# Coda-Research-Group/LearnedMetricIndex

Hardware: AMD Instinct MI355X
Metric: queries/sec @ recall@10, 768-d 10M index, 10k query batch (higher is better)
Workload: dtype f16 prefilter (f32 accumulate) + f32 exact re-rank; outputs identical to the all-f32 path

## Files before the change

learnedmetricindex_amd/csrc/lmi_handle.h:

```cpp
#pragma once
#include <hip/hip_runtime_api.h>

#include <cstdarg>
#include <cstdint>
#include <cstdio>
#include <string>
#include <utility>
#include <vector>

namespace {

thread_local std::string g_err;

int fail(const char* fmt, ...) {
    char buf[1024];
    va_list ap;
    va_start(ap, fmt);
    vsnprintf(buf, sizeof(buf), fmt, ap);
    va_end(ap);
    g_err = buf;
    return -1;
}

#define HIPCHK(expr)                                                                                \
// ... 152 lines not shown
    DevBuf aug_rows, q_aug, qn2;
    DevBuf stage;
    DevBuf wide;
    DevBuf q16_nav, q16_srch;
    bool q_srch_async = false;
    DevBuf rd_flag;
    DevBuf qdelta, qnorm, qscale, qfrag16, eps2, cand_cnt, cand_row, cand_s, fallback, pf_bound, nkeep, surv_row, rs_flag, rs_active;
    DevBuf grp_scratch;
    DevBuf x_log, x_ext, x_off, fb_list;
    unsigned x_cap = 0;
    DevBuf redo;
    size_t stamps_off = 0;
    int last_nslots = 0, last_nb = 0;
    long long last_ncols = 0;
    bool last_fast = false;
    static constexpr int PLAN_WORDS = 32;
    int32_t last_plan[PLAN_WORDS] = {};
    int32_t last_mlp_plan[PLAN_WORDS] = {};
    DevBuf act[2], xfrag, logits, order, q_nav, q_srch;
    DevBuf m, cb_start, item_base, part_base, stats, head, slot_local, slot_col, colmap, qfrag, grp, col_thr;
    DevBuf part_score, part_row, rank_d, rank_id, out_d, out_id, out_key;
    static constexpr int EV_RING = 128;
    hipEvent_t ev_ring[EV_RING][10] = {};
    bool valid_ring[EV_RING][10] = {};
    int ev_cur = 0;
    long long ev_calls = 0;
    hipEvent_t* ev = ev_ring[0];
    bool* ev_valid = valid_ring[0];
    long long h_stats[4] = {0, 0, 0, 0};
    bool stats_pending = false;
    DevBuf ts_ring;
    unsigned ts_mask[EV_RING] = {};
    unsigned long long* ts_set = nullptr;
    DevBuf fr_dbg;
    DevBuf cb_alloc, cb_bucket;
    unsigned* h_oflag = nullptr;
    int overflow_armed = 0;
    bool fr_bump_pending = false;
    DevBuf mut_pos, mut_ids, mut_list, mut_keep, mut_src, mut_stage, mut_word;
    lmi_index* parent = nullptr;
    int live_clones = 0;
};

struct lmi_index : DeviceFacts, Settings, Switches, Models, Buckets, CallState {};

static lmi_index* clone_handle(lmi_index* h) {
    lmi_index* c = new lmi_index();
    static_cast<DeviceFacts&>(*c) = *h;
    static_cast<Settings&>(*c) = *h;
    static_cast<Switches&>(*c) = *h;
    static_cast<Models&>(*c) = *h;
    static_cast<Buckets&>(*c) = *h;
    c->parent = h;
    h->live_clones++;
    return c;
}
```

learnedmetricindex_amd/csrc/lmi_host_debug.h:

```cpp
#pragma once
#include "lmi_host_mutate.h"
#include "lmi_host_search.h"

static int read_event_set(const hipEvent_t* ev, const bool* ev_valid, float* ms) {
    for (int i = 0; i < LMI_T_COUNT; ++i) ms[i] = 0.0f;
    auto span = [&](int a, int b, float* out) -> int {
        if (ev_valid[a] && ev_valid[b]) HIPCHK(hipEventElapsedTime(out, ev[a], ev[b]));
        return 0;
    };
    CHK(span(0, 1, &ms[LMI_T_INFERENCE]));
    CHK(span(1, 2, &ms[LMI_T_ROUTE]));
    CHK(span(2, 3, &ms[LMI_T_SCAN]));
    CHK(span(3, 4, &ms[LMI_T_MERGE]));
    CHK(span(2, 5, &ms[LMI_T_PF_SAMPLE]));
    CHK(span(5, 6, &ms[LMI_T_PF_EMIT]));
    CHK(span(6, 7, &ms[LMI_T_RESCORE]));
    CHK(span(7, 3, &ms[LMI_T_FALLBACK]));
    int first = ev_valid[0] ? 0 : 1;
    int last = ev_valid[4] ? 4 : 1;
    CHK(span(first, last, &ms[LMI_T_TOTAL]));
    return 0;
}

static void read_stamp_set(const lmi_index* h, const unsigned long long* v, unsigned mask, float* ms) {
// ... 154 lines not shown
    if (!h) return fail("lmi_debug_read_candidates: NULL handle");
    if (!h->last_fast) return fail("lmi_debug_read_candidates: the last scan did not use the prefilter");
    if (slot < 0 || slot >= h->last_nslots) return fail("lmi_debug_read_candidates: slot outside the last scan's %d", h->last_nslots);
    CHK(set_dev(h));
    HIPCHK(hipStreamSynchronize(h->stream));
    int col = -1;
    HIPCHK(hipMemcpy(&col, h->slot_col.as<int>() + slot, 4, hipMemcpyDeviceToHost));
    unsigned cnt = 0;
    float e2 = 0.0f, qs = 1.0f, xs[2] = {1.0f, 1.0f};
    if (col >= 0) {
        HIPCHK(hipMemcpy(&cnt, h->cand_cnt.as<unsigned>() + col, 4, hipMemcpyDeviceToHost));
        HIPCHK(hipMemcpy(&e2, h->eps2.as<float>() + col, 4, hipMemcpyDeviceToHost));
        HIPCHK(hipMemcpy(&qs, h->qscale.as<float>() + slot / h->last_nb, 4, hipMemcpyDeviceToHost));
        HIPCHK(hipMemcpy(xs, h->xscale.p, 8, hipMemcpyDeviceToHost));
        const unsigned n = std::min<unsigned>(std::min<unsigned>(cnt, (unsigned)PF_CAP), (unsigned)std::max(cap, 0));
        if (n && rows) HIPCHK(hipMemcpy(rows, h->cand_row.as<unsigned>() + (size_t)col * PF_CAP, (size_t)n * 4, hipMemcpyDeviceToHost));
        if (n && shat) HIPCHK(hipMemcpy(shat, h->cand_s.as<float>() + (size_t)col * PF_CAP, (size_t)n * 4, hipMemcpyDeviceToHost));
    }
    if (count) *count = col >= 0 ? (int)cnt : -1;
    if (eps2) *eps2 = e2;
    if (qscale) *qscale = qs;
    if (xscale) *xscale = xs[0];
    return 0;
}

extern "C" LMI_API int lmi_debug_peek(lmi_index* h, const char* name, void* dst, int64_t bytes) {
    if (!h || !name || !dst) return fail("lmi_debug_peek: NULL argument");
    CHK(set_dev(h));
    HIPCHK(hipStreamSynchronize(h->stream));
    DevBuf* b = nullptr;
    size_t off = 0;
    if (!strcmp(name, "pf_bound")) b = &h->pf_bound;
    if (!strcmp(name, "fr_dbg")) b = &h->fr_dbg;
    if (!strcmp(name, "pf_stamps")) { b = &h->pf_bound; off = h->stamps_off; }
    if (!strcmp(name, "cand_total")) {
        if (bytes != 8 || !h->last_fast) return fail("lmi_debug_peek: cand_total is 8 bytes after a prefilter scan");
        unsigned long long* d_acc = reinterpret_cast<unsigned long long*>(h->stats.as<long long>() + 2);
        HIPCHK(hipMemsetAsync(d_acc, 0, 8, h->stream));
        sum_u32_kernel<<<64, 256, 0, h->stream>>>(h->cand_cnt.as<unsigned>(), h->last_ncols, d_acc);
        HIPCHK(hipGetLastError());
        HIPCHK(hipStreamSynchronize(h->stream));
        HIPCHK(hipMemcpy(dst, d_acc, 8, hipMemcpyDeviceToHost));
        return 0;
    }
    if (!strcmp(name, "pf_redo")) b = &h->redo;
    if (!strcmp(name, "pf_fallback")) b = &h->fb_list;
    if (!b) return fail("lmi_debug_peek: unknown buffer '%s'", name);
    if (bytes < 0 || off + (size_t)bytes > b->cap) return fail("lmi_debug_peek: %lld bytes asked of a %zu-byte buffer", (long long)bytes, b->cap);
    if (bytes) HIPCHK(hipMemcpy(dst, static_cast<char*>(b->p) + off, (size_t)bytes, hipMemcpyDeviceToHost));
    return 0;
}

extern "C" LMI_API int lmi_scan_stats(lmi_index* h, double* flops, int64_t* pairs, int64_t* items) {
    if (!h) return fail("lmi_scan_stats: NULL handle");
    CHK(set_dev(h));
    if (h->stats_pending) {
        HIPCHK(hipStreamSynchronize(h->stream));
        HIPCHK(hipMemcpy(h->h_stats, h->stats.p, 32, hipMemcpyDeviceToHost));
        h->stats_pending = false;
    }
    if (pairs) *pairs = h->h_stats[0];
    if (items) *items = h->h_stats[1];
    if (flops) *flops = 2.0 * h->d * (double)h->h_stats[0];
    return 0;
}
```

learnedmetricindex_amd/csrc/lmi_host_model.h:

```cpp
#pragma once
#include "lmi_host.h"

static int pack_from_host(lmi_index* h, const float* src, int rows, int cols, int n_rb, int KG, DevBuf& dst) {
    CHK(h->stage.reserve((size_t)rows * cols * sizeof(float)));
    HIPCHK(hipMemcpyAsync(h->stage.p, src, (size_t)rows * cols * sizeof(float), hipMemcpyHostToDevice, h->stream));
    CHK(dst.reserve((size_t)n_rb * KG * 1024));
    long long total = (long long)n_rb * 32 * KG;
    pack_gather_kernel<<<cdiv(total, 256), 256, 0, h->stream>>>(h->stage.as<float>(), cols, nullptr, rows,
                                                               (long long)n_rb * 32, KG, dst.as<float4>());
    HIPCHK(hipGetLastError());
    HIPCHK(hipStreamSynchronize(h->stream));
    return 0;
}

static int pack_model(lmi_index* h, const char* who, int n_layers, const int* dims, const float* const* W, const float* const* b, Model& m) {
    h->desc_dirty = true;
    m.n_layers = 0;
    if (n_layers < 1 || n_layers > LMI_MAX_LAYERS) return fail("%s: n_layers %d out of range", who, n_layers);
    for (int i = 0; i <= n_layers; ++i)
        if (dims[i] < 1) return fail("%s: dims[%d] = %d", who, i, dims[i]);
    m.dims.assign(dims, dims + n_layers + 1);
    m.n_rb.assign(n_layers, 0);
    m.KG.assign(n_layers, 0);
    m.Wf.assign(n_layers, DevBuf());
// ... 134 lines not shown
        HIPCHK(hipMemcpy(h->d_child_model.p, child_model, (size_t)total * 4, hipMemcpyHostToDevice));
        HIPCHK(hipMemcpy(h->d_child_bucket.p, child_bucket, (size_t)total * 4, hipMemcpyHostToDevice));
    }
    h->tree_set = true;
    return 0;
}

struct FusedLds {
    bool ok = true;
    bool logits_lds = true;
    int s0 = 1, s1 = 1;
    int lds = 0;
};
static FusedLds fused_lds_plan(const std::vector<Model>& models) {
    FusedLds F;
    int w0 = 0, w1 = 0;
    for (const Model& M : models) {
        if (M.n_layers == 0) { F.ok = false; continue; }
        for (int i = 0; i < M.n_layers; ++i) {
            const int padded = M.n_rb[i] * 32;
            const bool last = i + 1 == M.n_layers;
            if (padded > FM_MAXH) { if (last) F.logits_lds = false; else F.ok = false; continue; }
            int& wref = (i & 1) ? w1 : w0;
            wref = std::max(wref, padded);
        }
    }
    F.s0 = w0 + 1;
    F.s1 = w1 + 1;
    F.lds = (2 * FM_COLS * FM_CHUNK_S + FM_COLS * F.s0 + FM_COLS * F.s1) * 4;
    if (F.lds > 160 * 1024 - 1024) F.ok = false;
    return F;
}

static int build_descs(lmi_index* h) {
    if (!h->desc_dirty) return 0;
    const int nm = (int)h->models.size();
    std::vector<ModelDesc> D(nm);
    for (int m = 0; m < nm; ++m) {
        const Model& M = h->models[m];
        ModelDesc& d = D[m];
        memset(&d, 0, sizeof(d));
        d.n_layers = M.n_layers;
        if (M.n_layers == 0) continue;
        for (int i = 0; i <= M.n_layers; ++i) d.dims[i] = M.dims[i];
        for (int i = 0; i < M.n_layers; ++i) {
            d.KG[i] = M.KG[i];
            d.W[i] = M.Wf[i].as<float4>();
            d.b[i] = M.bias[i].as<float>();
        }
    }
    const FusedLds F = fused_lds_plan(h->models);
    const bool ok = F.ok;
    h->fm_s0 = F.s0;
    h->fm_s1 = F.s1;
    h->fm_act0 = FM_COLS * h->fm_s0;
    h->fm_lds = F.lds;
    h->fm_ok = ok;
    h->fm_logits_lds = F.logits_lds ? 1 : 0;
    CHK(h->d_models.reserve(sizeof(ModelDesc) * nm));
    HIPCHK(hipMemcpy(h->d_models.p, D.data(), sizeof(ModelDesc) * nm, hipMemcpyHostToDevice));
    if (ok) {
        HIPCHK(hipFuncSetAttribute(reinterpret_cast<const void*>(&mlp_fused_kernel<FM_TOPK>), hipFuncAttributeMaxDynamicSharedMemorySize, h->fm_lds));
        HIPCHK(hipFuncSetAttribute(reinterpret_cast<const void*>(&mlp_fused_kernel<FM_PROBA>), hipFuncAttributeMaxDynamicSharedMemorySize, h->fm_lds));
        HIPCHK(hipFuncSetAttribute(reinterpret_cast<const void*>(&mlp_fused_kernel<FM_NAV>), hipFuncAttributeMaxDynamicSharedMemorySize, h->fm_lds));
        HIPCHK(hipFuncSetAttribute(reinterpret_cast<const void*>(&mlp_fused_kernel<FM_TOPK_STOP>), hipFuncAttributeMaxDynamicSharedMemorySize, h->fm_lds));
        HIPCHK(hipFuncSetAttribute(reinterpret_cast<const void*>(&mlp_fused_kernel<FM_NAV_MASS>), hipFuncAttributeMaxDynamicSharedMemorySize, h->fm_lds));
        HIPCHK(hipFuncSetAttribute(reinterpret_cast<const void*>(&mlp_fused_kernel<FM_TOPK_ROWS>), hipFuncAttributeMaxDynamicSharedMemorySize, h->fm_lds));
    }
    h->desc_dirty = false;
    return 0;
}

static void fused_base(lmi_index* h, const float* d_q, int nq, FusedParams& P) {
    memset(&P, 0, sizeof(P));
    P.models = h->d_models.as<ModelDesc>();
    P.n_models = (int)h->models.size();
    P.x = d_q;
    P.d = h->root().dims[0];
    P.nq = nq;
    P.s0 = h->fm_s0;
    P.s1 = h->fm_s1;
    P.act0_floats = h->fm_act0;
    P.logits_in_lds = h->fm_logits_lds;
}

struct MlpPlan {
    int fused = 0;
    int mode = -1;
    int grid = 0;
    int nq_head = 0;
    int layers_queries = 0;
};
static MlpPlan mlp_plan(int num_cus, int fused_mlp, bool fm_ok, bool logits_lds, int nq, bool proba, bool want_logits, const RankStop& stop) {
    MlpPlan P;
    const bool fill = cdiv(nq, FM_COLS) * 2 >= num_cus || proba || fused_mlp == 2;
    if (!(fused_mlp && fm_ok && fill)) {
        P.layers_queries = nq;
        return P;
    }
    P.fused = 1;
    P.mode = proba ? FM_PROBA : stop.rows > 0 ? FM_TOPK_ROWS : stop.mass > 0.0f ? FM_TOPK_STOP : FM_TOPK;
    P.grid = cdiv(nq, FM_COLS);
    P.nq_head = nq;
    const int rem = P.grid % num_cus;
    if (fused_mlp == 1 && !proba && !want_logits && logits_lds && P.grid > num_cus && rem > 0 && rem * 10 < num_cus * 3) {
        P.nq_head = (P.grid - rem) * FM_COLS;
        P.grid -= rem;
        P.layers_queries = nq - P.nq_head;
    }
    return P;
}
static int mlp_layer_cbw(int num_cus, int n_rb, int ncb) {
    const int rows = cdiv(n_rb, 4);
    return rows * cdiv(ncb, 4) >= 2 * num_cus ? 4 : rows * cdiv(ncb, 2) >= 2 * num_cus ? 2 : 1;
}
static int fused_vec_in(int d) { return (d & 3) == 0; }
// ... 87 lines not shown
}

static int mlp_enqueue(lmi_index* h, const float* d_q, int nq, int nb, int* d_order, float* d_logits_out, float* d_probs = nullptr) {
    RankStop stop;
    CHK(mlp_call_check(h, nb, d_probs != nullptr, "lmi_mlp_topk", stop));
    const int L = h->root().dims.back();
    CHK(build_descs(h));
    const float mass = stop.mass;
    const MlpPlan plan = mlp_plan(h->num_cus, h->fused_mlp, h->fm_ok, h->fm_logits_lds != 0, nq, d_probs != nullptr, d_logits_out != nullptr, stop);
    {
        FusedLds F;
        F.ok = h->fm_ok; F.logits_lds = h->fm_logits_lds != 0; F.s0 = h->fm_s0; F.s1 = h->fm_s1; F.lds = h->fm_lds;
        mlp_plan_record(h, F, plan, h->last_mlp_plan);
    }
    if (plan.fused) {
        const int grid = plan.grid, nq_head = plan.nq_head;
        FusedParams P;
        fused_base(h, d_q, nq_head, P);
        float* d_logits = d_logits_out;
        if (!h->fm_logits_lds && !d_logits) {
            CHK(h->logits.reserve((size_t)nq * L * 4));
            d_logits = h->logits.as<float>();
        }
        P.logits_out = d_logits;
        P.nb = nb;
        P.order = d_order;
        P.probs = d_probs;
        P.classes = d_order;
        P.ts = tsp(h, ST_MLP0);
        P.stop_mass = mass;
        P.nb_rows = stop.nb_rows;
        P.stop_rows = stop.rows;
        if (nq_head < nq) CHK(side_fork(h));
        if (plan.mode == FM_PROBA) mlp_fused_kernel<FM_PROBA><<<grid, 256, h->fm_lds, h->stream>>>(P);
        else if (plan.mode == FM_TOPK_ROWS) mlp_fused_kernel<FM_TOPK_ROWS><<<grid, 256, h->fm_lds, h->stream>>>(P);
        else if (plan.mode == FM_TOPK_STOP) mlp_fused_kernel<FM_TOPK_STOP><<<grid, 256, h->fm_lds, h->stream>>>(P);
        else mlp_fused_kernel<FM_TOPK><<<grid, 256, h->fm_lds, h->stream>>>(P);
        HIPCHK(hipGetLastError());
        h->last_mlp_plan[LMI_MLP_PLAN_VEC_IN] = fused_vec_in(P.d);
        h->last_mlp_plan[LMI_MLP_PLAN_IN_CHUNKS] = fused_in_chunks(h->root().KG[0]);
        if (nq_head < nq) {
            CHK(mlp_layers_enqueue(h, h->side, d_q + (size_t)nq_head * h->root().dims[0], nq - nq_head, nb, d_order + (size_t)nq_head * nb, nullptr, nullptr, stop));
            CHK(side_join(h));
        }
        if (!h->fm_logits_lds) {
            CHK(rank_enqueue(h, h->stream, d_logits, nq, L, nb, stop, d_order));
            if (d_probs) {
                softmax_ranked_kernel<<<cdiv(nq, 64), 64, 0, h->stream>>>(d_logits, d_order, nq, L, d_probs);
                HIPCHK(hipGetLastError());
                h->last_mlp_plan[LMI_MLP_PLAN_SOFTMAX_KERNEL] = 1;
            }
        }
        return 0;
    }
    return mlp_layers_enqueue(h, h->stream, d_q, nq, nb, d_order, d_logits_out, d_probs, stop);
}

extern "C" LMI_API int lmi_mlp_topk(lmi_index* h, const float* queries_nav, int nq, int nb, int32_t* bucket_order,
                            float* logits, int on_device) {
    if (!h) return fail("lmi_mlp_topk: NULL handle");
    if (nq < 0) return fail("lmi_mlp_topk: nq < 0");
    if (nq == 0) return 0;
    CHK(set_dev(h));
    if (h->root().n_layers == 0) return fail("lmi_mlp_topk: no MLP set (lmi_set_mlp)");
    const int L = h->root().dims.back();
    const void* d_q = nullptr;
    CHK(input_ptr(h, queries_nav, (size_t)nq * h->root().dims[0] * 4, on_device, h->q_nav, &d_q));
    int* d_order = bucket_order;
    float* d_logits = logits;
    if (!on_device) {
// ... 69 lines not shown
        CHK(h->nav_parent_mass.reserve((size_t)nq * 4));
        CHK(h->nav_cum.reserve((size_t)nq * 4));
    }
    if (with_rows) CHK(h->nav_rows.reserve((size_t)nq * 8));
    FillRanges Z;
    Z.count = 0;
    bool fill_ok = true;
    auto fill = [&](void* ptr, long long words, unsigned value) { fill_ok = Z.add(ptr, words, value) && fill_ok; };
    fill(h->pq_len.p, nq, 0u);
    fill(h->nav_len.p, nq, 0u);
    fill(d_slab, (long long)nq * nb, 0xFFFFFFFFu);
    fill(d_ent, (long long)nq * nb, 0xFFFFFFFFu);
    fill(h->nav_count.p, 2 * (nm + 1), 0u);
    if (with_mass) {
        fill(h->nav_cum.p, nq, 0u);
        fill(h->nav_parent_mass.p, nq, 0x3F800000u);
    }
    if (with_rows) fill(h->nav_rows.p, 2ll * nq, 0u);
    if (!fill_ok) return fail("internal: more than %d fill ranges queued (%s:%d)", FillRanges::MAXR, __FILE__, __LINE__);
    Z.ts = tsp(h, ST_MLP0);
    fill_ranges_kernel<<<h->num_cus * 2, 256, 0, h->stream>>>(Z);
    HIPCHK(hipGetLastError());
    FusedParams P;
    fused_base(h, d_q, nq, P);
    P.pq_prob = h->pq_prob.as<float>();
    P.pq_ent = h->pq_ent.as<int>();
    P.pq_len = h->pq_len.as<int>();
    P.cap = cap;
    P.child_offset = h->d_child_offset.as<int>();
    P.reverse = 1;
    if (with_mass) {
        P.pq_mass = h->pq_mass.as<float>();
        P.parent_mass = h->nav_parent_mass.as<float>();
        mlp_fused_kernel<FM_NAV_MASS><<<cdiv(nq, FM_COLS), 256, h->fm_lds, h->stream>>>(P);
    } else {
        mlp_fused_kernel<FM_NAV><<<cdiv(nq, FM_COLS), 256, h->fm_lds, h->stream>>>(P);
    }
    HIPCHK(hipGetLastError());
    P.reverse = 0;
    P.col_query = h->nav_colq.as<int>();
    NavParams N;
    N.nq = nq; N.nb = nb; N.cap = cap;
    N.pq_prob = P.pq_prob; N.pq_ent = P.pq_ent; N.pq_len = P.pq_len;
    N.child_model = h->d_child_model.as<int>();
    N.child_bucket = h->d_child_bucket.as<int>();
    N.out_len = h->nav_len.as<int>();
    N.out_slab = d_slab;
    N.out_ent = d_ent;
    N.col_query = h->nav_colq.as<int>();
    NavMass S;
    memset(&S, 0, sizeof(S));
    if (with_mass) {
        S.pq_mass = h->pq_mass.as<float>();
        S.cum = h->nav_cum.as<float>();
        S.parent_mass = h->nav_parent_mass.as<float>();
        S.mass = h->path_mass;
    }
    NavRows W;
    memset(&W, 0, sizeof(W));
    if (with_rows) {
        W.nb_rows = h->d_nb_rows.as<int>();
        W.acc = h->nav_rows.as<long long>();
        W.rows = h->stop_rows;
    }
    int* counts = h->nav_count.as<int>();
    const int max_steps = nm + 1;
    const bool all = nm <= NAV_ENQUEUE_ALL;
    const bool pop_lds = cap <= NAV_LDS_CAP;
    int h_active = 1;
    for (int it = 0; it < max_steps && h_active > 0;) {
        int last_par = 0;
        for (int k4 = 0; (all || k4 < 4) && it < max_steps; ++k4, ++it) {
            const int par = it & 1;
            N.node_count = counts + par * (nm + 1);
            N.active = counts + par * (nm + 1) + nm;
            N.prev_active = (all && it > 0) ? counts + (1 - par) * (nm + 1) + nm : nullptr;
            if (with_mass && with_rows) {
                if (pop_lds) nav_pop_lds_mass_rows_kernel<<<cdiv(nq, 64), 64, (size_t)cap * 64 * 8, h->stream>>>(N, S, W);
                else nav_pop_mass_rows_kernel<<<cdiv(nq, 256), 256, 0, h->stream>>>(N, S, W);
            } else if (with_rows) {
                if (pop_lds) nav_pop_lds_rows_kernel<<<cdiv(nq, 64), 64, (size_t)cap * 64 * 8, h->stream>>>(N, W);
                else nav_pop_rows_kernel<<<cdiv(nq, 256), 256, 0, h->stream>>>(N, W);
            } else if (with_mass) {
                if (pop_lds) nav_pop_lds_mass_kernel<<<cdiv(nq, 64), 64, (size_t)cap * 64 * 8, h->stream>>>(N, S);
                else nav_pop_mass_kernel<<<cdiv(nq, 256), 256, 0, h->stream>>>(N, S);
            } else {
                if (pop_lds) nav_pop_lds_kernel<<<cdiv(nq, 64), 64, (size_t)cap * 64 * 8, h->stream>>>(N);
                else nav_pop_kernel<<<cdiv(nq, 256), 256, 0, h->stream>>>(N);
            }
            HIPCHK(hipGetLastError());
            P.node_count = N.node_count;
            P.zero_counts = counts + (1 - par) * (nm + 1);
            P.n_zero = nm + 1;
            if (with_mass) mlp_fused_kernel<FM_NAV_MASS><<<cdiv(nq, FM_COLS) + nm, 256, h->fm_lds, h->stream>>>(P);
            else mlp_fused_kernel<FM_NAV><<<cdiv(nq, FM_COLS) + nm, 256, h->fm_lds, h->stream>>>(P);
            HIPCHK(hipGetLastError());
            last_par = par;
        }
        if (all) break;
        HIPCHK(hipMemcpyAsync(&h_active, counts + last_par * (nm + 1) + nm, 4, hipMemcpyDeviceToHost, h->stream));
        HIPCHK(hipStreamSynchronize(h->stream));
    }
    return 0;
}

extern "C" LMI_API int lmi_nav_order(lmi_index* h, const float* queries_nav, int nq, int nb, int32_t* slab_ids, int32_t* entries,
                             int on_device) {
    if (!h) return fail("lmi_nav_order: NULL handle");
    if (nq < 0 || nb < 1) return fail("lmi_nav_order: bad nq/n_buckets");
    if (nq == 0) return 0;
    CHK(nav_check(h, nq, nb, "lmi_nav_order"));
    const void* d_q = nullptr;
    CHK(input_ptr(h, queries_nav, (size_t)nq * h->root().dims[0] * 4, on_device, h->q_nav, &d_q));
    CHK(h->nav_slab.reserve((size_t)nq * nb * 4));
    CHK(h->nav_ent.reserve((size_t)nq * nb * 4));
    int* d_slab = on_device ? slab_ids : h->nav_slab.as<int>();
    int* d_ent = on_device ? entries : h->nav_ent.as<int>();
    begin_call(h);
    CHK(record(h, 0));
    CHK(nav_enqueue(h, static_cast<const float*>(d_q), nq, nb, d_slab, d_ent));
    CHK(record(h, 1));
    CHK(stamp_end(h, ST_MLP1));
    if (!on_device) CHK(copy_back(h, {{slab_ids, d_slab, (size_t)nq * nb * 4}, {entries, d_ent, (size_t)nq * nb * 4}}));
    return 0;
}
```

learnedmetricindex_amd/csrc/lmi_kernels.h:

```cpp
#pragma once
#include <hip/hip_runtime.h>
#include <stdint.h>

namespace lmi {

typedef float f32x16 __attribute__((ext_vector_type(16)));

constexpr int KPB = 10;
#ifndef LMI_SCAN_RB
#define LMI_SCAN_RB 1
#endif
constexpr int RB = LMI_SCAN_RB;
constexpr int TILE_ROWS = 128 * RB;
constexpr int TILE_COLS = 128;
constexpr int STAGE_G = 4;
constexpr int SCAN_LDS = 0;
constexpr unsigned NOROW = 0xFFFFFFFFu;
constexpr int NGRP = 8;

__device__ __forceinline__ int acc_row(int r, int h) { return (r & 3) + 8 * (r >> 2) + 4 * h; }

enum { ST_MLP0 = 0, ST_MLP1, ST_FRONT, ST_P1, ST_P2, ST_P2END, ST_TAIL, ST_FB, ST_MERGE, ST_END, ST_SCAN0, ST_SCAN1,
       ST_CLK_WALL, ST_CLK_CYC,
       ST_COUNT = 16 };
// ... 109 lines not shown
    unsigned char* __restrict__ dst = C.dst[blockIdx.y];
    const long long bytes = C.bytes[blockIdx.y], n16 = bytes >> 4;
    const long long stride = (long long)gridDim.x * blockDim.x;
    for (long long i = (long long)blockIdx.x * blockDim.x + threadIdx.x; i < n16; i += stride)
        reinterpret_cast<uint4*>(dst)[i] = reinterpret_cast<const uint4*>(src)[i];
    const long long t = (n16 << 4) + (long long)blockIdx.x * blockDim.x + threadIdx.x;
    if (t < bytes) dst[t] = src[t];
}

template <bool LAST, int CBW = 4>
__global__ __launch_bounds__(256) void mlp_layer_kernel(const float4* __restrict__ Wf,
                                                        const float* __restrict__ bias,
                                                        const float4* __restrict__ Xf, int KG, int n_rb,
                                                        int ncb, float* __restrict__ out, int KGn,
                                                        int nq, int L) {
    const int lane = threadIdx.x & 63, w = threadIdx.x >> 6, h = lane >> 5, c = lane & 31;
    const int rb = blockIdx.y * 4 + w;
    const int cb0 = blockIdx.x * CBW;
    if (rb >= n_rb) return;
    f32x16 acc[CBW];
#pragma unroll
    for (int r = 0; r < 16; ++r) {
        float bv = bias[rb * 32 + acc_row(r, h)];
#pragma unroll
        for (int n = 0; n < CBW; ++n) acc[n][r] = bv;
    }
    const float4* ap = Wf + (size_t)rb * KG * 64 + lane;
    const float4* bp[CBW];
#pragma unroll
    for (int n = 0; n < CBW; ++n) {
        int cb = cb0 + n < ncb ? cb0 + n : ncb - 1;
        bp[n] = Xf + (size_t)cb * KG * 64 + lane;
    }
    float4 a = ap[0];
    float4 b[CBW];
#pragma unroll
    for (int n = 0; n < CBW; ++n) b[n] = bp[n][0];
    for (int g = 0; g < KG; ++g) {
        const int gn = g + 1 < KG ? g + 1 : g;
        const float4 a_next = ap[(size_t)gn * 64];
        float4 b_next[CBW];
#pragma unroll
        for (int n = 0; n < CBW; ++n) b_next[n] = bp[n][(size_t)gn * 64];
        const float av[4] = {a.x, a.y, a.z, a.w};
#pragma unroll
        for (int s = 0; s < 4; ++s) {
#pragma unroll
            for (int n = 0; n < CBW; ++n) {
                const float bv = s == 0 ? b[n].x : s == 1 ? b[n].y : s == 2 ? b[n].z : b[n].w;
                acc[n] = __builtin_amdgcn_mfma_f32_32x32x2f32(av[s], bv, acc[n], 0, 0, 0);
            }
        }
        a = a_next;
#pragma unroll
        for (int n = 0; n < CBW; ++n) b[n] = b_next[n];
    }
#pragma unroll
    for (int n = 0; n < CBW; ++n) {
        const int cb = cb0 + n;
        if (cb >= ncb) continue;
        const int q = cb * 32 + c;
        if (LAST) {
            if (q < nq) {
#pragma unroll
                for (int r = 0; r < 16; ++r) {
                    int j = rb * 32 + acc_row(r, h);
                    if (j < L) out[(size_t)q * L + j] = acc[n][r];
                }
            }
        } else {
            float* o = out + ((size_t)cb * KGn) * 256;
#pragma unroll
            for (int qd = 0; qd < 4; ++qd) {
                float v0 = fmaxf(acc[n][4 * qd + 0], 0.0f), v1 = fmaxf(acc[n][4 * qd + 1], 0.0f);
                float v2 = fmaxf(acc[n][4 * qd + 2], 0.0f), v3 = fmaxf(acc[n][4 * qd + 3], 0.0f);
                float* og = o + (size_t)(rb * 4 + qd) * 256;
                *reinterpret_cast<float2*>(og + (0 * 32 + c) * 4 + 2 * h) = make_float2(v0, v2);
                *reinterpret_cast<float2*>(og + (1 * 32 + c) * 4 + 2 * h) = make_float2(v1, v3);
            }
        }
    }
}

__global__ __launch_bounds__(64) void rank_classes_kernel(const float* __restrict__ logits, int nq, int L,
                                                         int nb, int* __restrict__ order) {
    const int q = blockIdx.x, lane = threadIdx.x;
    if (q >= nq) return;
    const float* l = logits + (size_t)q * L;
    float pv = INFINITY;
// ... 1023 lines not shown
```

learnedmetricindex_amd/csrc/lmi_mlp_fused.h:

```cpp
#pragma once
#include "lmi_kernels.h"

namespace lmi {

constexpr int FM_MAXL = 8;
constexpr int FM_COLS = 32;
constexpr int FM_CHUNK = 96;
constexpr int FM_CHUNK_S = FM_CHUNK + 1;
constexpr int FM_MAXH = 512;
enum { FM_TOPK = 0, FM_PROBA = 1, FM_NAV = 2, FM_TOPK_STOP = 3, FM_NAV_MASS = 4, FM_TOPK_ROWS = 5 };

struct ModelDesc {
    int n_layers;
    int dims[FM_MAXL + 1];
    int KG[FM_MAXL];
    const float4* W[FM_MAXL];
    const float* b[FM_MAXL];
};

struct FusedParams {
    const ModelDesc* models;
    int n_models;
    const float* x;
    int d, nq;
    int s0, s1;
    int act0_floats;
    int logits_in_lds;
    const int* node_count;
    const int* col_query;
    int nb;
    int* order;
    float* logits_out;
    float* probs;
    int* classes;
    float* pq_prob;
    int* pq_ent;
    int* pq_len;
    int cap;
    const int* child_offset;
    int reverse;
    int* zero_counts;
    int n_zero;
    unsigned long long* ts;
    float stop_mass;
    float* pq_mass;
    const float* parent_mass;
    const int* nb_rows;
    long long stop_rows;
};

template <int MODE>
__global__ __launch_bounds__(256) void mlp_fused_kernel(FusedParams P) {
    extern __shared__ __attribute__((aligned(16))) float fm_smem[];
    __shared__ int s_hdr[4];
    __shared__ int s_q[FM_COLS];
    __shared__ float s_max[FM_COLS], s_sum[FM_COLS];
    const int tid = threadIdx.x, lane = tid & 63, h = lane >> 5, c = lane & 31;
    const int w = __builtin_amdgcn_readfirstlane(tid >> 6);
    ts_first(P.ts);
    if (tid == 0) {
        int model = -1, ncols = 0, first = 0;
        if (!P.node_count) {
            model = 0;
            first = blockIdx.x * FM_COLS;
            ncols = min(FM_COLS, P.nq - first);
        } else {
            int b = blockIdx.x;
            for (int m = 0; m < P.n_models; ++m) {
                const int cnt = P.node_count[m];
                const int cbs = (cnt + FM_COLS - 1) / FM_COLS;
                if (b < cbs) { model = m; first = b * FM_COLS; ncols = min(FM_COLS, cnt - first); break; }
                b -= cbs;
            }
        }
        s_hdr[0] = ncols > 0 ? model : -1;
        s_hdr[1] = ncols;
        s_hdr[2] = first;
    }
    if (P.zero_counts && blockIdx.x == 0)
        for (int i = tid; i < P.n_zero; i += 256) P.zero_counts[i] = 0;
    __syncthreads();
    const int model = s_hdr[0], ncols = s_hdr[1], first = s_hdr[2];
    if (model < 0) return;
    if (tid < FM_COLS)
        s_q[tid] = tid < ncols ? (P.node_count ? P.col_query[(size_t)model * P.nq + first + tid] : first + tid) : -1;
    __syncthreads();
    const ModelDesc& M = P.models[model];
    const int n_layers = M.n_layers;
    float* chunk0 = fm_smem;
    float* chunk1 = fm_smem + FM_COLS * FM_CHUNK_S;
    float* act0 = fm_smem + 2 * FM_COLS * FM_CHUNK_S;
    float* act1 = act0 + P.act0_floats;
    const int L = M.dims[n_layers];
    constexpr bool NAV = MODE == FM_NAV || MODE == FM_NAV_MASS;

    for (int li = 0; li < n_layers; ++li) {
        const int J = M.dims[li + 1];
        const int n_rb = (J + 31) >> 5;
        const int KG = M.KG[li];
        const bool last = li + 1 == n_layers;
        float* out = (li & 1) ? act1 : act0;
        const int So = (li & 1) ? P.s1 : P.s0;
        const float* in = (li & 1) ? act0 : act1;
        const int Si = (li & 1) ? P.s0 : P.s1;
        const bool out_lds = !last || P.logits_in_lds;
        typedef float f4v __attribute__((ext_vector_type(4)));
        typedef const __attribute__((address_space(1))) f4v* gf4;
        typedef const __attribute__((address_space(1))) float* gf1;
        const gf4 Wl = (gf4)M.W[li];
        const gf1 bl = (gf1)M.b[li];
        for (int pass = 0; pass * 16 < n_rb; ++pass) {
            int rb[4];
            bool ok[4];
            f32x16 acc[4];
#pragma unroll
            for (int j = 0; j < 4; ++j) {
                rb[j] = pass * 16 + 4 * j + w;
                ok[j] = rb[j] < n_rb;
#pragma unroll
                for (int r = 0; r < 16; ++r) acc[j][r] = bl[(ok[j] ? rb[j] : 0) * 32 + acc_row(r, h)];
            }
            gf4 ap[4];
#pragma unroll
            for (int j = 0; j < 4; ++j) ap[j] = Wl + (size_t)(ok[j] ? rb[j] : 0) * KG * 64 + lane;
            f4v aq0[4], aq1[4], aq2[4];
#pragma unroll
            for (int j = 0; j < 4; ++j) {
                aq0[j] = ap[j][0];
                aq1[j] = ap[j][(size_t)min(1, KG - 1) * 64];
                aq2[j] = ap[j][(size_t)min(2, KG - 1) * 64];
            }
#define FM_STEP(AQ, BNEXT, G)                                                                              \
            {                                                                                              \
                const float* bs_ = (BNEXT);   \
                const float n0 = bs_[0 + h], n1 = bs_[2 + h], n2 = bs_[4 + h], n3 = bs_[6 + h];            \
                _Pragma("unroll") for (int j = 0; j < 4; ++j) {                                            \
                    if (ok[j]) {                                                                           \
                        acc[j] = __builtin_amdgcn_mfma_f32_32x32x2f32(AQ[j].x, bq0, acc[j], 0, 0, 0);      \
                        acc[j] = __builtin_amdgcn_mfma_f32_32x32x2f32(AQ[j].y, bq1, acc[j], 0, 0, 0);      \
                        acc[j] = __builtin_amdgcn_mfma_f32_32x32x2f32(AQ[j].z, bq2, acc[j], 0, 0, 0);      \
                        acc[j] = __builtin_amdgcn_mfma_f32_32x32x2f32(AQ[j].w, bq3, acc[j], 0, 0, 0);      \
                    }                                                                                      \
                }                                                                                          \
                const int gn_ = min((G) + 3, KG - 1);                                                      \
                _Pragma("unroll") for (int j = 0; j < 4; ++j) AQ[j] = ap[j][(size_t)gn_ * 64];             \
                bq0 = n0; bq1 = n1; bq2 = n2; bq3 = n3;                                                    \
            }
#define FM_RANGE(BASE, G0, G1)                                                                             \
            {                                                                                              \
                int g_ = (G0);                                                                             \
                const float* bb_ = (BASE);                                                                 \
                const int last_ = ((G1) - (G0) - 1) * 8;                                                   \
                float bq0 = bb_[0 + h], bq1 = bb_[2 + h], bq2 = bb_[4 + h], bq3 = bb_[6 + h];              \
                int o_ = 0;                                                                                \
                for (; g_ + 3 <= (G1); g_ += 3, o_ += 24) {                                                \
                    FM_STEP(aq0, bb_ + min(o_ + 8, last_), g_)                                             \
                    FM_STEP(aq1, bb_ + min(o_ + 16, last_), g_ + 1)                                        \
                    FM_STEP(aq2, bb_ + min(o_ + 24, last_), g_ + 2)                                        \
                }                                                                                          \
                if (g_ < (G1)) FM_STEP(aq0, bb_ + min(o_ + 8, last_), g_)                                  \
                if (g_ + 1 < (G1)) FM_STEP(aq1, bb_ + min(o_ + 16, last_), g_ + 1)                         \
            }
            if (li == 0) {
                const int d = P.d;
                const int nck = (KG * 8 + FM_CHUNK - 1) / FM_CHUNK;
                const int row = tid >> 3, seg = tid & 7;
                const int qi = s_q[row];
                const float* src = P.x + (size_t)(qi < 0 ? 0 : qi) * d;
                const bool vec_ok = (d & 3) == 0;
                float4 st[3];
                auto fetch = [&](int ck) {
                    const int k0 = ck * FM_CHUNK + seg * 12;
                    if (vec_ok && (ck + 1) * FM_CHUNK <= d) {
#pragma unroll
                        for (int i = 0; i < 3; ++i) st[i] = *reinterpret_cast<const float4*>(src + k0 + 4 * i);
                    } else {
                        float e[12];
#pragma unroll
                        for (int i = 0; i < 12; ++i) e[i] = src[min(k0 + i, d - 1)];
#pragma unroll
                        for (int i = 0; i < 12; ++i) e[i] = k0 + i < d ? e[i] : 0.0f;
#pragma unroll
                        for (int i = 0; i < 3; ++i) st[i] = make_float4(e[4 * i], e[4 * i + 1], e[4 * i + 2], e[4 * i + 3]);
                    }
                    if (qi < 0) {
#pragma unroll
                        for (int i = 0; i < 3; ++i) st[i] = make_float4(0.f, 0.f, 0.f, 0.f);
                    }
                };
                auto put = [&](float* buf) {
                    float* dst = buf + row * FM_CHUNK_S + seg * 12;
#pragma unroll
                    for (int i = 0; i < 3; ++i) { dst[4 * i + 0] = st[i].x; dst[4 * i + 1] = st[i].y; dst[4 * i + 2] = st[i].z; dst[4 * i + 3] = st[i].w; }
                };
                fetch(0);
                put(chunk0);
                __syncthreads();
                for (int ck = 0; ck < nck; ++ck) {
                    const float* cur = (ck & 1) ? chunk1 : chunk0;
                    if (ck + 1 < nck) fetch(ck + 1);
                    const int g_end = min(KG, (ck + 1) * (FM_CHUNK / 8));
                    FM_RANGE(cur + c * FM_CHUNK_S, ck * (FM_CHUNK / 8), g_end)
                    if (ck + 1 < nck) put((ck & 1) ? chunk0 : chunk1);
                    __syncthreads();
                }
            } else {
                FM_RANGE(in + c * Si, 0, KG)
            }
#undef FM_RANGE
#undef FM_STEP
#pragma unroll
            for (int j = 0; j < 4; ++j) {
                if (!ok[j]) continue;
#pragma unroll
                for (int r = 0; r < 16; ++r) {
                    const int f = rb[j] * 32 + acc_row(r, h);
                    float v = acc[j][r];
                    if (!last) v = fmaxf(v, 0.0f);
                    if (out_lds) out[c * So + f] = v;
                    if (last && P.logits_out && c < ncols && f < L) P.logits_out[(size_t)s_q[c] * L + f] = v;
                }
            }
        }
        __syncthreads();
    }
    if (!P.logits_in_lds) return;
    const float* lg = ((n_layers - 1) & 1) ? act1 : act0;
    const int SL = ((n_layers - 1) & 1) ? P.s1 : P.s0;
    if (MODE == FM_PROBA || NAV) {
        if (tid < ncols) {
            const float* l = lg + tid * SL;
            float m = l[0];
            for (int j = 1; j < L; ++j) m = l[j] > m ? l[j] : m;
            float s = 0.0f;
            for (int j = 0; j < L; ++j) s += lmi_expf(l[j] - m);
            s_max[tid] = m;
            s_sum[tid] = s;
        }
        __syncthreads();
    }
    const int T = (MODE == FM_TOPK || MODE == FM_TOPK_STOP || MODE == FM_TOPK_ROWS) ? P.nb : L;
    const int col = w * 8 + (lane >> 3), sub = lane & 7;
    const bool live = col < ncols;
    const int q = s_q[live ? col : 0];
    const float* l = lg + (live ? col : 0) * SL;
    float sm = 0.0f, ss = 0.0f, cum = 0.0f;
    const bool rows_mass = MODE == FM_TOPK_ROWS && P.stop_mass > 0.0f;
    long long racc = 0;
    if (MODE == FM_TOPK_STOP || rows_mass) {
        sm = l[0];
        for (int j = sub; j < L; j += 8) {
            const float v = l[j];
            sm = v > sm ? v : sm;
        }
#pragma unroll
        for (int o = 4; o > 0; o >>= 1) {
            const float ov = __shfl_xor(sm, o);
            sm = ov > sm ? ov : sm;
        }
        for (int j0 = 0; j0 < L; j0 += 8) {
            const int j = j0 + sub;
            const float e = j < L ? lmi_expf(l[min(j, L - 1)] - sm) : 0.0f;
#pragma unroll
            for (int k = 0; k < 8; ++k) ss += __shfl(e, k, 8);
        }
    }
    int base = 0;
    if (NAV) base = P.pq_len[q];
    float pmass = 1.0f;
    if (MODE == FM_NAV_MASS) pmass = P.parent_mass[q];
    float pv = INFINITY;
    int pi = -1;
// ... 16 lines not shown
            if (MODE == FM_TOPK) {
                P.order[(size_t)q * P.nb + t] = cls;
            } else if (MODE == FM_TOPK_STOP) {
                P.order[(size_t)q * P.nb + t] = (t == 0 || cum < P.stop_mass) ? cls : -1;
                const float pr = cls >= 0 ? lmi_expf(l[cls] - sm) / ss : __builtin_nanf("");
                cum = t == 0 ? pr : cum + pr;
            } else if (MODE == FM_TOPK_ROWS) {
                const bool go = racc < P.stop_rows && (!rows_mass || cum < P.stop_mass);
                P.order[(size_t)q * P.nb + t] = (t == 0 || go) ? cls : -1;
                if (rows_mass) {
                    const float pr = cls >= 0 ? lmi_expf(l[cls] - sm) / ss : __builtin_nanf("");
                    cum = t == 0 ? pr : cum + pr;
                }
                if (cls >= 0) racc += P.nb_rows[cls];
            } else {
                const float pr = cls >= 0 ? lmi_expf(l[cls] - s_max[col]) / s_sum[col] : __builtin_nanf("");
                if (MODE == FM_PROBA) {
                    P.classes[(size_t)q * L + t] = cls;
                    P.probs[(size_t)q * L + t] = pr;
                } else {
                    const int pos = base + (P.reverse ? L - 1 - t : t);
                    if (pos < P.cap) {
                        P.pq_prob[(size_t)pos * P.nq + q] = pr;
                        P.pq_ent[(size_t)pos * P.nq + q] = cls >= 0 ? P.child_offset[model] + cls : -1;
                        if (MODE == FM_NAV_MASS) P.pq_mass[(size_t)pos * P.nq + q] = __fmul_rn(pmass, pr);
                    }
                }
            }
        }
        pv = bv;
        pi = bi;
    }
    if (NAV && sub == 0 && live) P.pq_len[q] = min(P.cap, base + L);
}

struct NavParams {
    int nq, nb, cap;
    float* pq_prob;
    int* pq_ent;
    const int* pq_len;
    const int* child_model;
    const int* child_bucket;
    int* out_len;
    int* out_slab;
    int* out_ent;
    int* node_count;
    int* col_query;
    int* active;
    const int* prev_active;
};
struct NavRows {
    const int* nb_rows;
    long long* acc;
    long long rows;
};
struct NavMass {
    const float* pq_mass;
    float* cum;
    float* parent_mass;
    float mass;
};

__device__ __forceinline__ void nav_push(const NavParams& P, int q, int my_cm) {
    const int lane = (int)__builtin_amdgcn_mbcnt_hi(~0u, __builtin_amdgcn_mbcnt_lo(~0u, 0u));
    unsigned long long todo = __ballot(my_cm >= 0);
    const int total = (int)__popcll(todo);
    if (total == 0) return;
// ... 35 lines not shown
```

Baseline: 2.091 million.

## Run fused MLP kernel with eight waves and deepen non-fused MLP prefetch

```diff
diff --git a/learnedmetricindex_amd/csrc/lmi_handle.h b/learnedmetricindex_amd/csrc/lmi_handle.h
--- a/learnedmetricindex_amd/csrc/lmi_handle.h
+++ b/learnedmetricindex_amd/csrc/lmi_handle.h
@@ -208,6 +208,7 @@
     DevBuf ts_ring;
     unsigned ts_mask[EV_RING] = {};
     unsigned long long* ts_set = nullptr;
+    DevBuf fm_stamps;
     DevBuf fr_dbg;
     DevBuf cb_alloc, cb_bucket;
     unsigned* h_oflag = nullptr;
diff --git a/learnedmetricindex_amd/csrc/lmi_host_debug.h b/learnedmetricindex_amd/csrc/lmi_host_debug.h
--- a/learnedmetricindex_amd/csrc/lmi_host_debug.h
+++ b/learnedmetricindex_amd/csrc/lmi_host_debug.h
@@ -210,6 +210,7 @@
     size_t off = 0;
     if (!strcmp(name, "pf_bound")) b = &h->pf_bound;
     if (!strcmp(name, "fr_dbg")) b = &h->fr_dbg;
+    if (!strcmp(name, "fm_stamps")) b = &h->fm_stamps;
     if (!strcmp(name, "pf_stamps")) { b = &h->pf_bound; off = h->stamps_off; }
     if (!strcmp(name, "cand_total")) {
         if (bytes != 8 || !h->last_fast) return fail("lmi_debug_peek: cand_total is 8 bytes after a prefilter scan");
diff --git a/learnedmetricindex_amd/csrc/lmi_host_model.h b/learnedmetricindex_amd/csrc/lmi_host_model.h
--- a/learnedmetricindex_amd/csrc/lmi_host_model.h
+++ b/learnedmetricindex_amd/csrc/lmi_host_model.h
@@ -190,6 +190,19 @@
     return F;
 }
 
+static int fused_waves(bool beside_chain) { return beside_chain ? 4 : 8; }
+template <int MODE>
+static void fused_launch(lmi_index* h, int grid, int waves, const FusedParams& P) {
+    if (waves == 8) mlp_fused_kernel<MODE, 8><<<grid, 512, h->fm_lds, h->stream>>>(P);
+    else mlp_fused_kernel<MODE, 4><<<grid, 256, h->fm_lds, h->stream>>>(P);
+}
+template <int MODE>
+static int fused_set_lds(int lds) {
+    HIPCHK(hipFuncSetAttribute(reinterpret_cast<const void*>(&mlp_fused_kernel<MODE, 4>), hipFuncAttributeMaxDynamicSharedMemorySize, lds));
+    HIPCHK(hipFuncSetAttribute(reinterpret_cast<const void*>(&mlp_fused_kernel<MODE, 8>), hipFuncAttributeMaxDynamicSharedMemorySize, lds));
+    return 0;
+}
+
 static int build_descs(lmi_index* h) {
     if (!h->desc_dirty) return 0;
     const int nm = (int)h->models.size();
@@ -218,13 +231,19 @@
     CHK(h->d_models.reserve(sizeof(ModelDesc) * nm));
     HIPCHK(hipMemcpy(h->d_models.p, D.data(), sizeof(ModelDesc) * nm, hipMemcpyHostToDevice));
     if (ok) {
-        HIPCHK(hipFuncSetAttribute(reinterpret_cast<const void*>(&mlp_fused_kernel<FM_TOPK>), hipFuncAttributeMaxDynamicSharedMemorySize, h->fm_lds));
-        HIPCHK(hipFuncSetAttribute(reinterpret_cast<const void*>(&mlp_fused_kernel<FM_PROBA>), hipFuncAttributeMaxDynamicSharedMemorySize, h->fm_lds));
-        HIPCHK(hipFuncSetAttribute(reinterpret_cast<const void*>(&mlp_fused_kernel<FM_NAV>), hipFuncAttributeMaxDynamicSharedMemorySize, h->fm_lds));
-        HIPCHK(hipFuncSetAttribute(reinterpret_cast<const void*>(&mlp_fused_kernel<FM_TOPK_STOP>), hipFuncAttributeMaxDynamicSharedMemorySize, h->fm_lds));
-        HIPCHK(hipFuncSetAttribute(reinterpret_cast<const void*>(&mlp_fused_kernel<FM_NAV_MASS>), hipFuncAttributeMaxDynamicSharedMemorySize, h->fm_lds));
-        HIPCHK(hipFuncSetAttribute(reinterpret_cast<const void*>(&mlp_fused_kernel<FM_TOPK_ROWS>), hipFuncAttributeMaxDynamicSharedMemorySize, h->fm_lds));
-    }
+        CHK(fused_set_lds<FM_TOPK>(h->fm_lds));
+        CHK(fused_set_lds<FM_PROBA>(h->fm_lds));
+        CHK(fused_set_lds<FM_NAV>(h->fm_lds));
+        CHK(fused_set_lds<FM_TOPK_STOP>(h->fm_lds));
+        CHK(fused_set_lds<FM_NAV_MASS>(h->fm_lds));
+        CHK(fused_set_lds<FM_TOPK_ROWS>(h->fm_lds));
+    }
+#ifdef LMI_FM_STAMPS
+    if (!h->fm_stamps.p) {
+        CHK(h->fm_stamps.reserve(FM_MAX_WAVES * FMS_SLOTS * 8));
+        HIPCHK(hipMemset(h->fm_stamps.p, 0, FM_MAX_WAVES * FMS_SLOTS * 8));
+    }
+#endif
     h->desc_dirty = false;
     return 0;
 }
@@ -240,6 +259,9 @@
     P.s1 = h->fm_s1;
     P.act0_floats = h->fm_act0;
     P.logits_in_lds = h->fm_logits_lds;
+#ifdef LMI_FM_STAMPS
+    P.stamps = h->fm_stamps.as<unsigned long long>();
+#endif
 }
 
 struct MlpPlan {
@@ -393,10 +415,11 @@
         P.nb_rows = stop.nb_rows;
         P.stop_rows = stop.rows;
         if (nq_head < nq) CHK(side_fork(h));
-        if (plan.mode == FM_PROBA) mlp_fused_kernel<FM_PROBA><<<grid, 256, h->fm_lds, h->stream>>>(P);
-        else if (plan.mode == FM_TOPK_ROWS) mlp_fused_kernel<FM_TOPK_ROWS><<<grid, 256, h->fm_lds, h->stream>>>(P);
-        else if (plan.mode == FM_TOPK_STOP) mlp_fused_kernel<FM_TOPK_STOP><<<grid, 256, h->fm_lds, h->stream>>>(P);
-        else mlp_fused_kernel<FM_TOPK><<<grid, 256, h->fm_lds, h->stream>>>(P);
+        const int waves = fused_waves(nq_head < nq);
+        if (plan.mode == FM_PROBA) fused_launch<FM_PROBA>(h, grid, waves, P);
+        else if (plan.mode == FM_TOPK_ROWS) fused_launch<FM_TOPK_ROWS>(h, grid, waves, P);
+        else if (plan.mode == FM_TOPK_STOP) fused_launch<FM_TOPK_STOP>(h, grid, waves, P);
+        else fused_launch<FM_TOPK>(h, grid, waves, P);
         HIPCHK(hipGetLastError());
         h->last_mlp_plan[LMI_MLP_PLAN_VEC_IN] = fused_vec_in(P.d);
         h->last_mlp_plan[LMI_MLP_PLAN_IN_CHUNKS] = fused_in_chunks(h->root().KG[0]);
@@ -532,9 +555,9 @@
     if (with_mass) {
         P.pq_mass = h->pq_mass.as<float>();
         P.parent_mass = h->nav_parent_mass.as<float>();
-        mlp_fused_kernel<FM_NAV_MASS><<<cdiv(nq, FM_COLS), 256, h->fm_lds, h->stream>>>(P);
+        fused_launch<FM_NAV_MASS>(h, cdiv(nq, FM_COLS), fused_waves(false), P);
     } else {
-        mlp_fused_kernel<FM_NAV><<<cdiv(nq, FM_COLS), 256, h->fm_lds, h->stream>>>(P);
+        fused_launch<FM_NAV>(h, cdiv(nq, FM_COLS), fused_waves(false), P);
     }
     HIPCHK(hipGetLastError());
     P.reverse = 0;
@@ -592,8 +615,8 @@
             P.node_count = N.node_count;
             P.zero_counts = counts + (1 - par) * (nm + 1);
             P.n_zero = nm + 1;
-            if (with_mass) mlp_fused_kernel<FM_NAV_MASS><<<cdiv(nq, FM_COLS) + nm, 256, h->fm_lds, h->stream>>>(P);
-            else mlp_fused_kernel<FM_NAV><<<cdiv(nq, FM_COLS) + nm, 256, h->fm_lds, h->stream>>>(P);
+            if (with_mass) fused_launch<FM_NAV_MASS>(h, cdiv(nq, FM_COLS) + nm, fused_waves(false), P);
+            else fused_launch<FM_NAV>(h, cdiv(nq, FM_COLS) + nm, fused_waves(false), P);
             HIPCHK(hipGetLastError());
             last_par = par;
         }
diff --git a/learnedmetricindex_amd/csrc/lmi_kernels.h b/learnedmetricindex_amd/csrc/lmi_kernels.h
--- a/learnedmetricindex_amd/csrc/lmi_kernels.h
+++ b/learnedmetricindex_amd/csrc/lmi_kernels.h
@@ -165,29 +165,33 @@
         int cb = cb0 + n < ncb ? cb0 + n : ncb - 1;
         bp[n] = Xf + (size_t)cb * KG * 64 + lane;
     }
-    float4 a = ap[0];
-    float4 b[CBW];
-#pragma unroll
-    for (int n = 0; n < CBW; ++n) b[n] = bp[n][0];
-    for (int g = 0; g < KG; ++g) {
-        const int gn = g + 1 < KG ? g + 1 : g;
-        const float4 a_next = ap[(size_t)gn * 64];
-        float4 b_next[CBW];
-#pragma unroll
-        for (int n = 0; n < CBW; ++n) b_next[n] = bp[n][(size_t)gn * 64];
-        const float av[4] = {a.x, a.y, a.z, a.w};
-#pragma unroll
-        for (int s = 0; s < 4; ++s) {
-#pragma unroll
-            for (int n = 0; n < CBW; ++n) {
-                const float bv = s == 0 ? b[n].x : s == 1 ? b[n].y : s == 2 ? b[n].z : b[n].w;
-                acc[n] = __builtin_amdgcn_mfma_f32_32x32x2f32(av[s], bv, acc[n], 0, 0, 0);
-            }
-        }
-        a = a_next;
-#pragma unroll
-        for (int n = 0; n < CBW; ++n) b[n] = b_next[n];
-    }
+    float4 a0 = ap[0], a1 = ap[(size_t)min(1, KG - 1) * 64], a2 = ap[(size_t)min(2, KG - 1) * 64];
+    float4 b0[CBW], b1[CBW], b2[CBW];
+#pragma unroll
+    for (int n = 0; n < CBW; ++n) {
+        b0[n] = bp[n][0];
+        b1[n] = bp[n][(size_t)min(1, KG - 1) * 64];
+        b2[n] = bp[n][(size_t)min(2, KG - 1) * 64];
+    }
+#define LMI_MLP_STEP(A, B, G)                                                                              \
+    {                                                                                                      \
+        _Pragma("unroll") for (int n = 0; n < CBW; ++n) acc[n] = __builtin_amdgcn_mfma_f32_32x32x2f32(A.x, B[n].x, acc[n], 0, 0, 0); \
+        _Pragma("unroll") for (int n = 0; n < CBW; ++n) acc[n] = __builtin_amdgcn_mfma_f32_32x32x2f32(A.y, B[n].y, acc[n], 0, 0, 0); \
+        _Pragma("unroll") for (int n = 0; n < CBW; ++n) acc[n] = __builtin_amdgcn_mfma_f32_32x32x2f32(A.z, B[n].z, acc[n], 0, 0, 0); \
+        _Pragma("unroll") for (int n = 0; n < CBW; ++n) acc[n] = __builtin_amdgcn_mfma_f32_32x32x2f32(A.w, B[n].w, acc[n], 0, 0, 0); \
+        const size_t gn_ = (size_t)min((G) + 3, KG - 1) * 64;                                              \
+        A = ap[gn_];                                                                                       \
+        _Pragma("unroll") for (int n = 0; n < CBW; ++n) B[n] = bp[n][gn_];                                 \
+    }
+    int g = 0;
+    for (; g + 3 <= KG; g += 3) {
+        LMI_MLP_STEP(a0, b0, g)
+        LMI_MLP_STEP(a1, b1, g + 1)
+        LMI_MLP_STEP(a2, b2, g + 2)
+    }
+    if (g < KG) LMI_MLP_STEP(a0, b0, g)
+    if (g + 1 < KG) LMI_MLP_STEP(a1, b1, g + 1)
+#undef LMI_MLP_STEP
 #pragma unroll
     for (int n = 0; n < CBW; ++n) {
         const int cb = cb0 + n;
diff --git a/learnedmetricindex_amd/csrc/lmi_mlp_fused.h b/learnedmetricindex_amd/csrc/lmi_mlp_fused.h
--- a/learnedmetricindex_amd/csrc/lmi_mlp_fused.h
+++ b/learnedmetricindex_amd/csrc/lmi_mlp_fused.h
@@ -8,6 +8,7 @@
 constexpr int FM_CHUNK = 96;
 constexpr int FM_CHUNK_S = FM_CHUNK + 1;
 constexpr int FM_MAXH = 512;
+constexpr int FM_MAX_WAVES = 8;
 enum { FM_TOPK = 0, FM_PROBA = 1, FM_NAV = 2, FM_TOPK_STOP = 3, FM_NAV_MASS = 4, FM_TOPK_ROWS = 5 };
 
 struct ModelDesc {
@@ -47,10 +48,35 @@
     const float* parent_mass;
     const int* nb_rows;
     long long stop_rows;
+#ifdef LMI_FM_STAMPS
+    unsigned long long* stamps;
+#endif
 };
 
-template <int MODE>
-__global__ __launch_bounds__(256) void mlp_fused_kernel(FusedParams P) {
+enum { FMS_HEAD = 0,
+       FMS_FETCH = 1,
+       FMS_MFMA0 = 2,
+       FMS_PUT = 3,
+       FMS_BAR = 4,
+       FMS_LATER = 5,
+       FMS_WB = 6,
+       FMS_SOFTMAX = 7, FMS_RANK = 8, FMS_BLOCKS = 9, FMS_SLOTS = 16 };
+#ifdef LMI_FM_STAMPS
+#define FM_STAMP(PH) { const unsigned long long t_ = __builtin_readcyclecounter(); st_acc[PH] += t_ - st_last; st_last = t_; }
+#define FM_STAMPS_FLUSH()                                                                                  \
+    if (P.stamps && lane == 0) {                                                                           \
+        for (int ph_ = 0; ph_ < FMS_BLOCKS; ++ph_) atomicAdd(&P.stamps[w * FMS_SLOTS + ph_], st_acc[ph_]); \
+        atomicAdd(&P.stamps[w * FMS_SLOTS + FMS_BLOCKS], 1ull);                                            \
+    }
+#else
+#define FM_STAMP(PH)
+#define FM_STAMPS_FLUSH()
+#endif
+
+template <int MODE, int WAVES>
+__global__ __launch_bounds__(64 * WAVES) void mlp_fused_kernel(FusedParams P) {
+    static_assert(WAVES == 4 || WAVES == 8, "the row fetch and the ranking epilogue are written for waves 0-3");
+    constexpr int FM_ACCS = 16 / WAVES;
     extern __shared__ __attribute__((aligned(16))) float fm_smem[];
     __shared__ int s_hdr[4];
     __shared__ int s_q[FM_COLS];
@@ -58,6 +84,10 @@
     const int tid = threadIdx.x, lane = tid & 63, h = lane >> 5, c = lane & 31;
     const int w = __builtin_amdgcn_readfirstlane(tid >> 6);
     ts_first(P.ts);
+#ifdef LMI_FM_STAMPS
+    unsigned long long st_acc[FMS_BLOCKS] = {};
+    unsigned long long st_last = __builtin_readcyclecounter();
+#endif
     if (tid == 0) {
         int model = -1, ncols = 0, first = 0;
         if (!P.node_count) {
@@ -78,7 +108,7 @@
         s_hdr[2] = first;
     }
     if (P.zero_counts && blockIdx.x == 0)
-        for (int i = tid; i < P.n_zero; i += 256) P.zero_counts[i] = 0;
+        for (int i = tid; i < P.n_zero; i += 64 * WAVES) P.zero_counts[i] = 0;
     __syncthreads();
     const int model = s_hdr[0], ncols = s_hdr[1], first = s_hdr[2];
     if (model < 0) return;
@@ -110,40 +140,48 @@
         const gf4 Wl = (gf4)M.W[li];
         const gf1 bl = (gf1)M.b[li];
         for (int pass = 0; pass * 16 < n_rb; ++pass) {
-            int rb[4];
-            bool ok[4];
-            f32x16 acc[4];
-#pragma unroll
-            for (int j = 0; j < 4; ++j) {
-                rb[j] = pass * 16 + 4 * j + w;
+            int rb[FM_ACCS];
+            bool ok[FM_ACCS];
+            f32x16 acc[FM_ACCS];
+#pragma unroll
+            for (int j = 0; j < FM_ACCS; ++j) {
+                rb[j] = pass * 16 + WAVES * j + w;
                 ok[j] = rb[j] < n_rb;
 #pragma unroll
                 for (int r = 0; r < 16; ++r) acc[j][r] = bl[(ok[j] ? rb[j] : 0) * 32 + acc_row(r, h)];
             }
-            gf4 ap[4];
-#pragma unroll
-            for (int j = 0; j < 4; ++j) ap[j] = Wl + (size_t)(ok[j] ? rb[j] : 0) * KG * 64 + lane;
-            f4v aq0[4], aq1[4], aq2[4];
-#pragma unroll
-            for (int j = 0; j < 4; ++j) {
+            gf4 ap[FM_ACCS];
+#pragma unroll
+            for (int j = 0; j < FM_ACCS; ++j) ap[j] = Wl + (size_t)(ok[j] ? rb[j] : 0) * KG * 64 + lane;
+            f4v aq0[FM_ACCS], aq1[FM_ACCS], aq2[FM_ACCS];
+#pragma unroll
+            for (int j = 0; j < FM_ACCS; ++j) {
                 aq0[j] = ap[j][0];
                 aq1[j] = ap[j][(size_t)min(1, KG - 1) * 64];
                 aq2[j] = ap[j][(size_t)min(2, KG - 1) * 64];
             }
+            FM_STAMP(FMS_HEAD)
 #define FM_STEP(AQ, BNEXT, G)                                                                              \
             {                                                                                              \
                 const float* bs_ = (BNEXT);   \
                 const float n0 = bs_[0 + h], n1 = bs_[2 + h], n2 = bs_[4 + h], n3 = bs_[6 + h];            \
-                _Pragma("unroll") for (int j = 0; j < 4; ++j) {                                            \
-                    if (ok[j]) {                                                                           \
-                        acc[j] = __builtin_amdgcn_mfma_f32_32x32x2f32(AQ[j].x, bq0, acc[j], 0, 0, 0);      \
-                        acc[j] = __builtin_amdgcn_mfma_f32_32x32x2f32(AQ[j].y, bq1, acc[j], 0, 0, 0);      \
-                        acc[j] = __builtin_amdgcn_mfma_f32_32x32x2f32(AQ[j].z, bq2, acc[j], 0, 0, 0);      \
-                        acc[j] = __builtin_amdgcn_mfma_f32_32x32x2f32(AQ[j].w, bq3, acc[j], 0, 0, 0);      \
+                if (WAVES == 8 && ok[FM_ACCS - 1]) {                                                       \
+                    _Pragma("unroll") for (int j = 0; j < FM_ACCS; ++j) acc[j] = __builtin_amdgcn_mfma_f32_32x32x2f32(AQ[j].x, bq0, acc[j], 0, 0, 0); \
+                    _Pragma("unroll") for (int j = 0; j < FM_ACCS; ++j) acc[j] = __builtin_amdgcn_mfma_f32_32x32x2f32(AQ[j].y, bq1, acc[j], 0, 0, 0); \
+                    _Pragma("unroll") for (int j = 0; j < FM_ACCS; ++j) acc[j] = __builtin_amdgcn_mfma_f32_32x32x2f32(AQ[j].z, bq2, acc[j], 0, 0, 0); \
+                    _Pragma("unroll") for (int j = 0; j < FM_ACCS; ++j) acc[j] = __builtin_amdgcn_mfma_f32_32x32x2f32(AQ[j].w, bq3, acc[j], 0, 0, 0); \
+                } else {                                                                                   \
+                    _Pragma("unroll") for (int j = 0; j < (WAVES == 8 ? FM_ACCS - 1 : FM_ACCS); ++j) {       \
+                        if (ok[j]) {                                                                       \
+                            acc[j] = __builtin_amdgcn_mfma_f32_32x32x2f32(AQ[j].x, bq0, acc[j], 0, 0, 0);  \
+                            acc[j] = __builtin_amdgcn_mfma_f32_32x32x2f32(AQ[j].y, bq1, acc[j], 0, 0, 0);  \
+                            acc[j] = __builtin_amdgcn_mfma_f32_32x32x2f32(AQ[j].z, bq2, acc[j], 0, 0, 0);  \
+                            acc[j] = __builtin_amdgcn_mfma_f32_32x32x2f32(AQ[j].w, bq3, acc[j], 0, 0, 0);  \
+                        }                                                                                  \
                     }                                                                                      \
                 }                                                                                          \
                 const int gn_ = min((G) + 3, KG - 1);                                                      \
-                _Pragma("unroll") for (int j = 0; j < 4; ++j) AQ[j] = ap[j][(size_t)gn_ * 64];             \
+                _Pragma("unroll") for (int j = 0; j < FM_ACCS; ++j) AQ[j] = ap[j][(size_t)gn_ * 64];       \
                 bq0 = n0; bq1 = n1; bq2 = n2; bq3 = n3;                                                    \
             }
 #define FM_RANGE(BASE, G0, G1)                                                                             \
@@ -164,7 +202,8 @@
             if (li == 0) {
                 const int d = P.d;
                 const int nck = (KG * 8 + FM_CHUNK - 1) / FM_CHUNK;
-                const int row = tid >> 3, seg = tid & 7;
+                const bool feeder = WAVES == 4 || w < 4;
+                const int row = (tid & 255) >> 3, seg = tid & 7;
                 const int qi = s_q[row];
                 const float* src = P.x + (size_t)(qi < 0 ? 0 : qi) * d;
                 const bool vec_ok = (d & 3) == 0;
@@ -193,24 +232,34 @@
 #pragma unroll
                     for (int i = 0; i < 3; ++i) { dst[4 * i + 0] = st[i].x; dst[4 * i + 1] = st[i].y; dst[4 * i + 2] = st[i].z; dst[4 * i + 3] = st[i].w; }
                 };
-                fetch(0);
-                put(chunk0);
+                if (feeder) {
+                    fetch(0);
+                    FM_STAMP(FMS_FETCH)
+                    put(chunk0);
+                    FM_STAMP(FMS_PUT)
+                }
                 __syncthreads();
+                FM_STAMP(FMS_BAR)
                 for (int ck = 0; ck < nck; ++ck) {
                     const float* cur = (ck & 1) ? chunk1 : chunk0;
-                    if (ck + 1 < nck) fetch(ck + 1);
+                    if (feeder && ck + 1 < nck) fetch(ck + 1);
+                    FM_STAMP(FMS_FETCH)
                     const int g_end = min(KG, (ck + 1) * (FM_CHUNK / 8));
                     FM_RANGE(cur + c * FM_CHUNK_S, ck * (FM_CHUNK / 8), g_end)
-                    if (ck + 1 < nck) put((ck & 1) ? chunk0 : chunk1);
+                    FM_STAMP(FMS_MFMA0)
+                    if (feeder && ck + 1 < nck) put((ck & 1) ? chunk0 : chunk1);
+                    FM_STAMP(FMS_PUT)
                     __syncthreads();
+                    FM_STAMP(FMS_BAR)
                 }
             } else {
                 FM_RANGE(in + c * Si, 0, KG)
+                FM_STAMP(FMS_LATER)
             }
 #undef FM_RANGE
 #undef FM_STEP
 #pragma unroll
-            for (int j = 0; j < 4; ++j) {
+            for (int j = 0; j < FM_ACCS; ++j) {
                 if (!ok[j]) continue;
 #pragma unroll
                 for (int r = 0; r < 16; ++r) {
@@ -223,8 +272,12 @@
             }
         }
         __syncthreads();
-    }
-    if (!P.logits_in_lds) return;
+        FM_STAMP(FMS_WB)
+    }
+    if (!P.logits_in_lds) {
+        FM_STAMPS_FLUSH()
+        return;
+    }
     const float* lg = ((n_layers - 1) & 1) ? act1 : act0;
     const int SL = ((n_layers - 1) & 1) ? P.s1 : P.s0;
     if (MODE == FM_PROBA || NAV) {
@@ -238,6 +291,11 @@
             s_sum[tid] = s;
         }
         __syncthreads();
+    }
+    FM_STAMP(FMS_SOFTMAX)
+    if (WAVES > 4 && w >= 4) {
+        FM_STAMPS_FLUSH()
+        return;
     }
     const int T = (MODE == FM_TOPK || MODE == FM_TOPK_STOP || MODE == FM_TOPK_ROWS) ? P.nb : L;
     const int col = w * 8 + (lane >> 3), sub = lane & 7;
@@ -320,7 +378,11 @@
         pi = bi;
     }
     if (NAV && sub == 0 && live) P.pq_len[q] = min(P.cap, base + L);
+    FM_STAMP(FMS_RANK)
+    FM_STAMPS_FLUSH()
 }
+#undef FM_STAMP
+#undef FM_STAMPS_FLUSH
 
 struct NavParams {
     int nq, nb, cap;
```

After: 2.078 million. About the same (-0.6%).
